# mx-mark/VideoTransformer-pytorch

Hardware: AMD Instinct MI355X
Metric: clips/sec TimeSformer-B divided_space_time 8x3x224x224 fwd+bwd (whole job) (higher is better)
Workload: dtype bf16

## Files before the change

### videotransformer-pytorch_amd/csrc/gemm_nt.hip

```cpp
#include "gemm_common.h"

namespace vtx {

constexpr int BK16 = 64;

__global__ __launch_bounds__(NT_THREADS) void gemm_nt_bf16_kernel(
    int M, int N, int K, const bf16raw* __restrict__ A, long lda, vtx_rowmap amap,
    const bf16raw* __restrict__ B, long ldb, int tiles_n, EpiParams ep) {
  extern __shared__ __attribute__((aligned(16))) char smem[];
  bf16raw* As = reinterpret_cast<bf16raw*>(smem);
  bf16raw* Bs = As + 2 * BM * BK16;
  const int tid = threadIdx.x, lane = tid & 63, wave = tid >> 6;
  const int wm = wave >> 1, wn = wave & 1;
  const int nwg = gridDim.x;
  const int tile = xcd_remap(blockIdx.x, nwg);
  const int tm = tile / tiles_n, tn = tile - tm * tiles_n;
  const int m0 = tm * BM, n0 = tn * BN;

  const int lc = tid & 7, lr = tid >> 3;
  const bf16raw* ap[4];
  const bf16raw* bp[4];
  int lds_off[4];
#pragma unroll
  for (int it = 0; it < 4; ++it) {
// ... 291 lines not shown
constexpr int PP_RING_BYTES = 2 * PP_BUF * 2;
constexpr int PP_STG_LD = 64;
constexpr int PP_LDS_BYTES = PP_RING_BYTES + 8 * 16 * PP_STG_LD * 4;
constexpr int PP_GRID = 256;

__device__ inline void lgkm0() { asm volatile("s_waitcnt lgkmcnt(0)" ::: "memory"); }

enum { PRE_NONE = 0, PRE_RES = 1, PRE_DGELU = 2, PRE_MUL = 3 };
template <bool EPI2, int PRE, bool HAS_SC, bool HAS_ACT, bool CONT, bool ROLL = false>
__global__ __launch_bounds__(PP_THREADS, 2) void gemm_nt_bf16_pp_kernel(
    int M, int N, int K, const bf16raw* __restrict__ A, long lda, vtx_rowmap amap,
    const bf16raw* __restrict__ B, long ldb, int tiles_n, int tiles_total, int CG, int* __restrict__ tile_ctr,
    long long* __restrict__ trace, int dbg, EpiParams ep) {
  extern __shared__ __attribute__((aligned(16))) char smem[];
  bf16raw* lds = reinterpret_cast<bf16raw*>(smem);
  amap.tab = nullptr;
  const int tid = threadIdx.x, lane = tid & 63;
  const int wave = __builtin_amdgcn_readfirstlane(tid >> 6);
  const int wr = wave >> 2, wc = wave & 3;
  float* stg = reinterpret_cast<float*>(smem + PP_RING_BYTES) + wave * 16 * PP_STG_LD;
  const int nk = K / PP_BK;
  int trace_tile = 0;
  auto stamp = [&](int e) {
    if (trace != nullptr && tid == 0 && trace_tile < 8) {
      long long* slot = trace + ((long)blockIdx.x * 8 + trace_tile) * 16;
      slot[e] = (long long)__builtin_amdgcn_s_memrealtime();
      if (e == 1 || e == 2) slot[7 + e] = (long long)__builtin_amdgcn_s_memtime();
    }
  };

// ... 19 lines not shown
  auto publish = [&](int v) -> int {
    if (tid == 0) *bcast = v;
    lgkm0();
    __builtin_amdgcn_s_barrier();
    const int t = *bcast;
    lgkm0();
    __builtin_amdgcn_s_barrier();
    return __builtin_amdgcn_readfirstlane(t);
  };
  auto next_tile = [&]() -> int {
    int v = 0;
    if (tid == 0) v = atomicAdd(my_ctr, 1);
    return publish(v);
  };
  static_assert(!CONT || EPI2, "the continuous flows belong to the read-ahead epilogue");
  constexpr bool CF = CONT && PRE == PRE_NONE;
  constexpr bool PF = CONT && PRE != PRE_NONE;
  const char* abase = nullptr;
  const char* bbase = nullptr;
  unsigned off[4][2];
  int m0 = 0, n0 = 0;
  int m0s = 0, n0s = 0;
  int par = 0;
  auto set_tile = [&](int t, long koff) {
    const int grp_tiles = nrow * CG;
    const int g = t / grp_tiles;
    const int wg = min(CG, tiles_n - g * CG);
    const int r = t - g * grp_tiles;
    const int rr = r / wg, cc = r - rr * wg;
    const int tm = rlo + rr, tn = g * CG + cc;
    m0s = tm * PP_BM; n0s = tn * PP_BN;
    const TileMap am = make_tile_map(amap, m0s);
// ... 98 lines not shown
      PP_READ_A(buf, 3);                                                                               \
      H3_                                                                                              \
      lgkm0();                                                                                         \
      PP_BAR();                                                                                        \
      PP_MMA_H(2, 1, fb1, ISS_(1, kt + 2, e2), M3W_, M3B_);                                            \
      PP_BAR();                                                                                        \
                                 \
      if (W4_) { if (w2) { if (X4_) wait_vmcnt<8 + NST>(); else if (R4_) wait_vmcnt<10>(); else wait_vmcnt<8>(); } else if (w1) wait_vmcnt<4>(); } \
      H4_                                                                                              \
      PP_BAR();                                                                                        \
      PP_MMA_H(2, 0, fb0, ISS_(2, kt + 2, e2), M4W_, M4B_);                                            \
      PP_BAR();                                                                                        \
    }
#define PP_ISS_COND(kind_, ktv_, ex_) if (ex_) issue(kind_, ktv_)
#define PP_ISS_ALWAYS(kind_, ktv_, ex_) issue(kind_, ktv_)
#define PP_ISS_PRE(kind_, ktv_, ex_) if (ex_) issue(kind_, ktv_); else pre_slot(kind_, ktv_)

  typedef __attribute__((address_space(3))) char lds_char;
  const unsigned slot_rd = (unsigned)(unsigned long)(lds_char*)(smem + PP_RING_BYTES);
  const unsigned bias_rd = (unsigned)(unsigned long)(lds_char*)(reinterpret_cast<char*>(stg) + 256 + (lane & 31) * 4);
  constexpr int NST = HAS_ACT ? 32 : 16;
  constexpr int NSR = NST / 4;
  bool relax = false;
  bool prev_rolled = false;
  int t = next_tile();
  const int tend = xcount;
  if (t >= tend) { check_out(); return; }
  int t_next = tend, t_nn = tend;
  if constexpr (CF) t_next = next_tile();
  int pending = 0;
  if (EPI2 && !CF && tid == 0) pending = atomicAdd(my_ctr, 1);
  set_tile(t, 0);
  m0 = m0s; n0 = n0s;
  prologue();
  while (true) {
    f32x16 acc[4][2];
#pragma unroll
    for (int i = 0; i < 4; ++i)
#pragma unroll
      for (int j = 0; j < 2; ++j)
#pragma unroll
        for (int r = 0; r < 16; ++r) acc[i][j][r] = 0.f;
    bf16x8 fa[2][4], fb0[4], fb1[4];
    const bool more_c = CF && t_next < tend;
    const int em0 = m0 + wr * 128, en0 = n0 + wc * 64;
    const int tile_m0 = m0;
    TileMap cm;
    unsigned ldcb = 0, lean_skipb = 0;
    bool lean = false;
    [[maybe_unused]] bool rolled = false;
    int lean_lb = 0;
    const char* lean_cb = nullptr;
    [[maybe_unused]] __amdgpu_buffer_rsrc_t lean_rsrc;
    float bcol[2] = {0.f, 0.f};
    auto epi_head = [&]() {
      cm = make_tile_map(ep.cmap, tile_m0);
      ldcb = (unsigned)ep.ldc * 2u;
      const long skipb64 = (long)cm.skip * (long)ldcb;
      lean = CONT && (dbg == 0 || dbg == 5 || dbg == 6) && em0 + 127 < ep.M && en0 + 63 < ep.N && (ep.split_row <= 0 || em0 + 127 < ep.split_row) &&
// ... 48 lines not shown
      _Pragma("unroll") for (int u = 0; u < 2; ++u) {                                                   \
        const unsigned sel = u ? 0x07060302u : 0x05040100u;                                             \
        u32x4 o;                                                                                        \
        o[0] = __builtin_amdgcn_perm(pl_w0[1], pl_w0[0], sel);                                          \
        o[1] = __builtin_amdgcn_perm(pl_w0[3], pl_w0[2], sel);                                          \
        o[2] = __builtin_amdgcn_perm(pl_w1[1], pl_w1[0], sel);                                          \
        o[3] = __builtin_amdgcn_perm(pl_w1[3], pl_w1[2], sel);                                          \
        const unsigned voff = pl_v0 + (u ? ldcb : 0u) + ((2 * pl_p2 + u >= lean_lb - 16 * (p_)) ? lean_skipb : 0u); \
         \
         \
        if constexpr (ROLL) __builtin_amdgcn_raw_buffer_store_b128(o, lean_rsrc, voff + (unsigned)(16 * (p_)) * ldcb, 0, 2); \
        else st16_nt_b(base, voff, o);                                                                  \
      }                                                                                                 \
    }
    constexpr bool ROLLK = ROLL;
    static_assert(!ROLL || (CF && VTX_PP_BF16_STAGE && PRE == PRE_NONE && !HAS_SC && !HAS_ACT), "rolling: the plain continuous flow only");
    stamp(0);
    if (relax) wait_vmcnt<10 + NST>(); else wait_vmcnt<10>();
    PP_BAR();
    stamp(1);
    if (wr == 1) PP_BAR();
    if constexpr (CF) {
      auto bias_dma = [&]() {
        if (ep.bias) {
          const int c = n0 + wc * 64 + lane;
          __builtin_amdgcn_global_load_lds((const __attribute__((address_space(1))) void*)(ep.bias + (c < ep.N ? c : 0)),
                                           (__attribute__((address_space(3))) void*)(stg + 64), 4, 0, 0);
        }
        if constexpr (HAS_SC) {
#pragma unroll
          for (int h = 0; h < 2; ++h) {
            int ml = m0 + wr * 128 + h * 64 + lane;
            if (ml >= ep.M) ml = ep.M - 1;
            const bool split = ep.split_row > 0 && ml >= ep.split_row;
            const unsigned q1 = fast_div((unsigned)ml, ep.rs_magic1, ep.rs_shift1);
            const unsigned q2 = fast_div((unsigned)ml, ep.rs_magic2, ep.rs_shift2);
            const int idx = split ? (ml - ep.split_row) : (int)q1 * ep.rs_m1 + (ml - (int)q2 * ep.rs_d2) * ep.rs_m2;
// ... 38 lines not shown
                      , PP_PF(0) PP_PW(0, 1) PP_PR();,
                      PP_PWAIT(0);, PP_PF(2) PP_PW(1, 1) PP_PR();)
        } else {
          PP_KTILE_XH(true, true, true, true, true, PP_ISS_ALWAYS, PP_CF_H1, PP_CF_H2;, PP_CF_H3, PP_CF_H4,
                      relax && kt < 2, relax && kt == 0, relax && kt == 0, prev_rolled && kt == 1, false, , , , )
        }
#undef PP_CF_H1
#undef PP_CF_H2
#undef PP_CF_H3
#undef PP_CF_H4
      } else {
        for (; kt < nk; ++kt) {
          PP_KTILE(kt + 1 < nk, kt + 2 < nk, kt + 1 < nk, kt + 2 < nk, true, PP_ISS_COND, if (kt == 0) bias_dma();, , , )
        }
      }
    } else if constexpr (PF) {
      constexpr bool pres = PRE == PRE_RES;
      const int pen = n0 + wc * 64 + (lane & 7) * 8;
      const unsigned penc2 = pen < ep.N ? (unsigned)pen * 2u : 0u;
      const unsigned pld2 = (unsigned)(pres ? ep.ldr : ep.ld_dgelu) * 2u;
      const int lastv = min(ep.M - 1, (pres && ep.split_row > 0) ? ep.split_row - 1 : 0x7fffffff);
      const int m0c = min(m0, lastv);
      const TileMap prm = make_tile_map(ep.rmap, m0c);
      const long pfirst = pres ? tile_map_row_u(prm, ep.rmap, m0c) : (long)m0c;
      const char* pbase = reinterpret_cast<const char*>(pres ? ep.R : ep.dgelu_in) + pfirst * (long)pld2;
      const int pbl = (pres && ep.rmap.grp > 0) ? prm.bound - m0c : 0x7fffffff;
      const int pskip = pres ? prm.skip : 0;
      const int plast = lastv - m0c;
      const int pl0 = (m0 - m0c) + wr * 128 + (lane >> 3);
      auto pre_piece = [&](int j, bf16raw* dst) {
        const int l = min(pl0 + 8 * j, plast);
        const int lr = l + (l >= pbl ? pskip : 0);
        const char* b = pbase;
        asm volatile("" : "+s"(b));
        dma16_nt(reinterpret_cast<const bf16raw*>(b + ((unsigned)lr * pld2 + penc2)), dst);
      };
      auto pre_slot = [&](int kind, int ktv) {
        const int s = (ktv - nk) * 4 + kind;
        bf16raw* dst = lds + ((ktv & 1) ^ par) * PP_BUF + kind * PP_REGION + wave * 1024;
        pre_piece(2 * s, dst);
        pre_piece(2 * s + 1, dst + 512);
        if (s == 6) {
          bf16raw* dst7 = lds + ((ktv & 1) ^ par) * PP_BUF + 3 * PP_REGION + wave * 1024;
          pre_piece(14, dst7);
          pre_piece(15, dst7 + 512);
        }
      };
      for (int kt = 0; kt < nk; ++kt) {
        PP_KTILE(kt + 1 < nk, kt + 2 < nk, true, true, kt + 1 < nk, PP_ISS_PRE, , , , )
      }
    } else {
      for (int kt = 0; kt < nk; ++kt) {
        PP_KTILE(kt + 1 < nk, kt + 2 < nk, kt + 1 < nk, kt + 2 < nk, true, PP_ISS_COND, , , , )
      }
    }
    if (wr == 0) PP_BAR();
    stamp(2);
    if constexpr (!EPI2) {
      t = next_tile();
      const bool more = t < tend;
      if (more) { set_tile(t, 0); m0 = m0s; n0 = n0s; prologue(); }
#define PP_EPI(mi_, half_)                                                                              \
      {                                                                                                 \
        const int col = lane & 31, rhalf = (lane >> 5) * 4;                                             \
        _Pragma("unroll") for (int ni = 0; ni < 2; ++ni) _Pragma("unroll") for (int r = 0; r < 8; ++r)  \
            stg[((r & 3) + 8 * (r >> 2) + rhalf) * PP_STG_LD + ni * 32 + col] = acc[mi_][ni][8 * (half_) + r]; \
        lgkm0();                                                                                        \
        __builtin_amdgcn_wave_barrier();                                                                \
        epilogue<bf16raw, 16, 2, PP_STG_LD>(ep, stg, em0 + (mi_) * 32 + (half_) * 16, en0, lane);       \
        lgkm0();                                                                                        \
        __builtin_amdgcn_wave_barrier();                                                                \
      }
      PP_EPI(0, 0) PP_EPI(0, 1) PP_EPI(1, 0) PP_EPI(1, 1) PP_EPI(2, 0) PP_EPI(2, 1) PP_EPI(3, 0) PP_EPI(3, 1)
#undef PP_EPI
      if (!more) break;
    } else {
      bool more = more_c;
      if constexpr (!CF) {
        t = publish(pending);
        more = t < tend;
      }
      stamp(3);
      int le = lane;
      asm volatile("" : "+v"(le));
      const int en = en0 + (le & 7) * 8;
      const bool col_ok = en < ep.N;
      const int enc = col_ok ? en : 0;
      const int er = em0 + (le >> 3);
      constexpr bool HAS_PRE = PRE != PRE_NONE, pre_res = PRE == PRE_RES;
      bf16raw* const pre_lds = lds + wave * (128 * 64);
      if (!rolled) epi_head();
      if constexpr (HAS_PRE && !PF) {
        const bf16raw* const pre_base = reinterpret_cast<const bf16raw*>(pre_res ? ep.R : ep.dgelu_in);
        const long pre_ld = pre_res ? ep.ldr : ep.ld_dgelu;
        const TileMap rm = make_tile_map(ep.rmap, tile_m0);
        const int row_last = ep.M - 1;
#pragma unroll
        for (int j = 0; j < 16; ++j) {
          int ml = er + 8 * j;
          const bool past = ml > row_last;
          if (past) ml = row_last;
          long rr = ml;
          if (pre_res) {
            const bool split = ep.split_row > 0 && ml >= ep.split_row;
            rr = split ? 0 : (ep.r_period > 0 ? (long)(ml % ep.r_period) : (past ? map_row(ep.rmap, ml) : tile_map_row(rm, ep.rmap, ml)));
          }
          dma16(pre_base + rr * pre_ld + enc, pre_lds + j * 512);
        }
      }
      if (ep.bias && !rolled) {
        if constexpr (CF) {
          asm volatile("ds_read_b32 %0, %2\n\tds_read_b32 %1, %2 offset:128\n\ts_waitcnt lgkmcnt(0)"
                       : "=&v"(bcol[0]), "=&v"(bcol[1]) : "v"(bias_rd) : "memory");
        } else {
#pragma unroll
          for (int ni = 0; ni < 2; ++ni) {
            const int c = en0 + ni * 32 + (le & 31);
            bcol[ni] = ep.bias[c < ep.N ? c : 0];
          }
        }
      }
      float sc[8][2];
      float scl[2] = {0.f, 0.f};
      if constexpr (HAS_SC && CF) {
        if (lean) {
          const unsigned scl_rd = (unsigned)(unsigned long)(lds_char*)(reinterpret_cast<char*>(stg) + 512 + le * 4);
          asm volatile("ds_read_b32 %0, %2\n\tds_read_b32 %1, %2 offset:256\n\ts_waitcnt lgkmcnt(0)"
                       : "=&v"(scl[0]), "=&v"(scl[1]) : "v"(scl_rd) : "memory");
        } else {
        const unsigned sc_rd = (unsigned)(unsigned long)(lds_char*)(reinterpret_cast<char*>(stg) + 512 + (le >> 3) * 4);
        asm volatile("ds_read_b32 %0, %16\n\tds_read_b32 %1, %16 offset:32\n\tds_read_b32 %2, %16 offset:64\n\t"
                     "ds_read_b32 %3, %16 offset:96\n\tds_read_b32 %4, %16 offset:128\n\tds_read_b32 %5, %16 offset:160\n\t"
                     "ds_read_b32 %6, %16 offset:192\n\tds_read_b32 %7, %16 offset:224\n\tds_read_b32 %8, %16 offset:256\n\t"
                     "ds_read_b32 %9, %16 offset:288\n\tds_read_b32 %10, %16 offset:320\n\tds_read_b32 %11, %16 offset:352\n\t"
                     "ds_read_b32 %12, %16 offset:384\n\tds_read_b32 %13, %16 offset:416\n\tds_read_b32 %14, %16 offset:448\n\t"
                     "ds_read_b32 %15, %16 offset:480\n\ts_waitcnt lgkmcnt(0)"
                     : "=&v"(sc[0][0]), "=&v"(sc[0][1]), "=&v"(sc[1][0]), "=&v"(sc[1][1]), "=&v"(sc[2][0]), "=&v"(sc[2][1]),
                       "=&v"(sc[3][0]), "=&v"(sc[3][1]), "=&v"(sc[4][0]), "=&v"(sc[4][1]), "=&v"(sc[5][0]), "=&v"(sc[5][1]),
                       "=&v"(sc[6][0]), "=&v"(sc[6][1]), "=&v"(sc[7][0]), "=&v"(sc[7][1])
                     : "v"(sc_rd) : "memory");
        }
      }
      if constexpr (HAS_SC && !CF) {
        auto scale_of = [&](int ml) -> float {
          if (ml >= ep.M) ml = ep.M - 1;
          const bool split = ep.split_row > 0 && ml >= ep.split_row;
          const unsigned q1 = fast_div((unsigned)ml, ep.rs_magic1, ep.rs_shift1);
          const unsigned q2 = fast_div((unsigned)ml, ep.rs_magic2, ep.rs_shift2);
          return ep.row_scale[split ? (ml - ep.split_row) : (int)q1 * ep.rs_m1 + (ml - (int)q2 * ep.rs_d2) * ep.rs_m2];
        };
        if (lean) {
          scl[0] = scale_of(em0 + le);
          scl[1] = scale_of(em0 + 64 + le);
        } else {
#pragma unroll
          for (int p = 0; p < 8; ++p)
#pragma unroll
            for (int u = 0; u < 2; ++u) sc[p][u] = scale_of(er + 16 * p + 8 * u);
        }
      }
      if constexpr (!CF) {
        if (more && tid == 0) pending = atomicAdd(my_ctr, 1);
        asm volatile("s_waitcnt vmcnt(0)" ::: "memory");
        stamp(4);
        asm volatile("" : "+v"(bcol[0]));
        asm volatile("" : "+v"(bcol[1]));
        if constexpr (HAS_SC) {
#pragma unroll
          for (int p = 0; p < 8; ++p) { asm volatile("" : "+v"(sc[p][0])); asm volatile("" : "+v"(sc[p][1])); }
          asm volatile("" : "+v"(scl[0])); asm volatile("" : "+v"(scl[1]));
        }
        if constexpr (!HAS_PRE) {
          if (more) { set_tile(t, 0); m0 = m0s; n0 = n0s; prologue(); }
        }
        if constexpr (PF) {
          if (more) set_tile(t, (long)nk * (PP_BK * 2));
        }
      }
      stamp(5);
      const unsigned stg_rd = (unsigned)(unsigned long)(lds_char*)(reinterpret_cast<char*>(stg) +
                                                                    ((le >> 3) * PP_STG_LD + (le & 7) * 8) * 4);
      const unsigned pre_rd = (unsigned)(unsigned long)(lds_char*)(reinterpret_cast<char*>(pre_lds) + le * 16);
      const unsigned pf_rd = (unsigned)(unsigned long)(lds_char*)(reinterpret_cast<char*>(lds + wave * 1024) + le * 16);
      const int pa = (nk & 1) ^ par;
#define PP_EPI2(p_, mi_, half_)                                                                         \
      {                                                                                                 \
        const int col = le & 31, rhalf = (le >> 5) * 4;                                             \
        if (dbg != 3) {                                                                                 \
        _Pragma("unroll") for (int ni = 0; ni < 2; ++ni) _Pragma("unroll") for (int r = 0; r < 8; ++r)  \
            stg[((r & 3) + 8 * (r >> 2) + rhalf) * PP_STG_LD + ni * 32 + col] = acc[mi_][ni][8 * (half_) + r] + bcol[ni]; \
        } else { stg[le] = acc[mi_][0][8 * (half_)] + acc[mi_][1][8 * (half_) + 7]; }                 \
        lgkm0();                                                                                        \
        __builtin_amdgcn_wave_barrier();                                                                \
        f32x4 s00, s01, s10, s11;                                                                       \
        u32x4 pre[2];                                                                                   \
        if constexpr (HAS_PRE) {                                                                        \
          const unsigned prd__ = PF ? pf_rd + (unsigned)((((p_) < 4 ? pa : pa ^ 1) * PP_BUF + ((p_) & 3) * PP_REGION) * 2) \
                                    : pre_rd + 2 * (p_) * 1024;                                         \
          asm volatile("ds_read_b128 %0, %6\n\tds_read_b128 %1, %6 offset:16\n\t"                       \
                       "ds_read_b128 %2, %6 offset:2048\n\tds_read_b128 %3, %6 offset:2064\n\t"         \
                       "ds_read_b128 %4, %7\n\tds_read_b128 %5, %7 offset:1024\n\t"                     \
                       "s_waitcnt lgkmcnt(0)"                                                           \
                       : "=&v"(s00), "=&v"(s01), "=&v"(s10), "=&v"(s11), "=&v"(pre[0]), "=&v"(pre[1])   \
                       : "v"(stg_rd), "v"(prd__) : "memory");                                           \
        } else                                                                                            \
          asm volatile("ds_read_b128 %0, %4\n\tds_read_b128 %1, %4 offset:16\n\t"                       \
                       "ds_read_b128 %2, %4 offset:2048\n\tds_read_b128 %3, %4 offset:2064\n\t"         \
                       "s_waitcnt lgkmcnt(0)"                                                           \
                       : "=&v"(s00), "=&v"(s01), "=&v"(s10), "=&v"(s11) : "v"(stg_rd) : "memory");      \
        __builtin_amdgcn_sched_barrier(0);                                                              \
        float v[2][8];                                                                                  \
        _Pragma("unroll") for (int j = 0; j < 4; ++j) {                                                 \
          v[0][j] = s00[j]; v[0][4 + j] = s01[j]; v[1][j] = s10[j]; v[1][4 + j] = s11[j];               \
        }                                                                                               \
        _Pragma("unroll") for (int u = 0; u < 2; ++u) {                                                 \
          const int m = er + 16 * (p_) + 8 * u;                                                         \
          const bool ok = col_ok && m < ep.M && dbg != 2;                                               \
          const bool split = ep.split_row > 0 && m >= ep.split_row;                                     \
          if constexpr (HAS_ACT) {                                                                      \
            if (ep.act == 2) {                               \
              float gp[8];                                                                              \
              _Pragma("unroll") for (int j = 0; j < 8; ++j) gelu_erf_both(v[u][j], v[u][j], gp[j]);     \
              if (ok) PP_ST8(reinterpret_cast<bf16raw*>(ep.C2) + (long)m * ep.ldc2 + en, gp);        \
            } else {                                                                                    \
              if (ep.C2 && ok) store8(reinterpret_cast<bf16raw*>(ep.C2) + (long)m * ep.ldc2 + en, v[u]); \
              _Pragma("unroll") for (int j = 0; j < 8; ++j) v[u][j] = gelu_erf(v[u][j]);                \
            }                                                                                           \
          }                                                                                             \
          if constexpr (PRE == PRE_MUL) {                          \
            const uint32_t w[4] = {pre[u][0], pre[u][1], pre[u][2], pre[u][3]};                         \
            _Pragma("unroll") for (int j = 0; j < 4; ++j) {                                             \
              v[u][2 * j] *= __uint_as_float(w[j] << 16);                                               \
              v[u][2 * j + 1] *= __uint_as_float(w[j] & 0xffff0000u);                                   \
            }                                                                                           \
          }                                                                                             \
          if constexpr (PRE == PRE_DGELU) {                                                             \
            const uint32_t w[4] = {pre[u][0], pre[u][1], pre[u][2], pre[u][3]};                         \
            _Pragma("unroll") for (int j = 0; j < 4; ++j) {                                             \
              v[u][2 * j] *= gelu_erf_grad(__uint_as_float(w[j] << 16));                                \
              v[u][2 * j + 1] *= gelu_erf_grad(__uint_as_float(w[j] & 0xffff0000u));                    \
            }                                                                                           \
          }                                                                                             \
          if constexpr (HAS_SC) { _Pragma("unroll") for (int j = 0; j < 8; ++j) v[u][j] *= sc[p_][u]; } \
          if (pre_res && !split) {                                                                      \
            const uint32_t w[4] = {pre[u][0], pre[u][1], pre[u][2], pre[u][3]};                         \
            _Pragma("unroll") for (int j = 0; j < 4; ++j) {                                             \
              v[u][2 * j] += __uint_as_float(w[j] << 16);                                               \
              v[u][2 * j + 1] += __uint_as_float(w[j] & 0xffff0000u);                                   \
            }                                                                                           \
          }                                                                                             \
          if (ok) {                                                                                     \
            if (split) store8(reinterpret_cast<bf16raw*>(ep.Csplit) + (long)(m - ep.split_row) * ep.ldsplit + en, v[u]); \
            else PP_ST8(reinterpret_cast<bf16raw*>(ep.C) + tile_map_row(cm, ep.cmap, m) * ep.ldc + en, v[u]); \
          }                                                                                             \
        }                                                                                               \
        if constexpr (PF) {                         \
          if ((p_) < 7 && more) issue((p_) & 3, nk + ((p_) >> 2));                                      \
        }                                                                                               \
      }
      constexpr bool PAIRS = VTX_PP_BF16_STAGE && PRE == PRE_NONE && !HAS_SC && !HAS_ACT;
      const unsigned stg_wr0 = (unsigned)(unsigned long)(lds_char*)(reinterpret_cast<char*>(stg)) ;
      if (lean) {
        int ln = le;
        asm volatile("" : "+v"(ln));
        if constexpr (PAIRS) {
          if (rolled) {
            PP_PWAIT(0); PP_PF(3)
          } else {
            pl_setup();
            PP_PW(0, 0) PP_PR();
            PP_PW(0, 1) PP_PWAIT(4); PP_PF(0) PP_PR();
            PP_PW(1, 0) PP_PWAIT(4); PP_PF(1) PP_PR();
// ... 3 lines not shown
          PP_PW(2, 0) PP_PR();
          PP_PW(2, 1) PP_PWAIT(4); PP_PF(4) PP_PR();
          PP_PW(3, 0) PP_PWAIT(4); PP_PF(5) PP_PR();
          PP_PW(3, 1) PP_PWAIT(4); PP_PF(6) PP_PR();
          PP_PWAIT(0); PP_PF(7)
        } else {
          const unsigned wa0 = stg_wr0 + (unsigned)(((ln >> 5) * 256 + (ln & 31)) * 4), wa1 = wa0 + 512 * 4;
          const unsigned vf0 = (unsigned)(ln >> 3) * ldcb + (unsigned)(ln & 7) * 16u;
          const unsigned ldc2b = (unsigned)ep.ldc2 * 2u;
          const unsigned vg0 = (unsigned)(ln >> 3) * ldc2b + (unsigned)(ln & 7) * 16u;
          const char* const lean_c2b = reinterpret_cast<const char*>(ep.C2) + ((long)em0 * ep.ldc2 + en0) * 2;
          f32x4 s00, s01, s10, s11;
          u32x4 pre[2];
          float scu[2] = {1.f, 1.f};
          const unsigned bp_addr = (unsigned)(ln >> 3) * 4u;
#define PP_LW(mi_, half_) if (ep.bias) { PP_LW_(mi_, half_, true) } else { PP_LW_(mi_, half_, false) }
#define PP_LW_(mi_, half_, B_)                                                                          \
          {                                                                                             \
            _Pragma("unroll") for (int kk = 0; kk < 2; ++kk) _Pragma("unroll") for (int ni = 0; ni < 2; ++ni) \
            _Pragma("unroll") for (int r2 = 0; r2 < 2; ++r2) {                                          \
              f32x2 xy = mk2(acc[mi_][ni][8 * (half_) + 4 * kk + 2 * r2], acc[mi_][ni][8 * (half_) + 4 * kk + 2 * r2 + 1]); \
              if (B_) { const f32x2 b2 = mk2(bcol[ni], bcol[ni]); xy = xy + b2; }                       \
              const float x = xy[0];                                                                    \
              const float y = xy[1];                                                                    \
              const unsigned wa = kk ? wa1 : wa0;                                                       \
              if (ni == 0 && r2 == 0) asm volatile("ds_write2_b32 %0, %1, %2 offset1:64" :: "v"(wa), "v"(x), "v"(y) : "memory"); \
              if (ni == 0 && r2 == 1) asm volatile("ds_write2_b32 %0, %1, %2 offset0:128 offset1:192" :: "v"(wa), "v"(x), "v"(y) : "memory"); \
              if (ni == 1 && r2 == 0) asm volatile("ds_write2_b32 %0, %1, %2 offset0:32 offset1:96" :: "v"(wa), "v"(x), "v"(y) : "memory"); \
              if (ni == 1 && r2 == 1) asm volatile("ds_write2_b32 %0, %1, %2 offset0:160 offset1:224" :: "v"(wa), "v"(x), "v"(y) : "memory"); \
            }                                                                                           \
          }
#define PP_LR(p_)                                                                                       \
          if constexpr (HAS_PRE) {                                                                      \
            const unsigned prd__ = PF ? pf_rd + (unsigned)((((p_) < 4 ? pa : pa ^ 1) * PP_BUF + ((p_) & 3) * PP_REGION) * 2) \
                                      : pre_rd + 2 * (p_) * 1024;                                       \
            asm volatile("ds_read_b128 %0, %6\n\tds_read_b128 %1, %6 offset:16\n\t"                     \
                         "ds_read_b128 %2, %6 offset:2048\n\tds_read_b128 %3, %6 offset:2064\n\t"       \
                         "ds_read_b128 %4, %7\n\tds_read_b128 %5, %7 offset:1024"                       \
                         : "=&v"(s00), "=&v"(s01), "=&v"(s10), "=&v"(s11), "=&v"(pre[0]), "=&v"(pre[1]) \
                         : "v"(stg_rd), "v"(prd__) : "memory");                                         \
          } else                                                                                        \
            asm volatile("ds_read_b128 %0, %4\n\tds_read_b128 %1, %4 offset:16\n\t"                     \
                         "ds_read_b128 %2, %4 offset:2048\n\tds_read_b128 %3, %4 offset:2064"           \
                         : "=&v"(s00), "=&v"(s01), "=&v"(s10), "=&v"(s11) : "v"(stg_rd) : "memory");      \
          if constexpr (HAS_SC)                         \
            asm volatile("ds_bpermute_b32 %0, %2, %3 offset:%4\n\tds_bpermute_b32 %1, %2, %3 offset:%5"   \
                         : "=&v"(scu[0]), "=&v"(scu[1]) : "v"(bp_addr), "v"((p_) < 4 ? scl[0] : scl[1]),   \
                           "n"(((16 * (p_)) & 63) * 4), "n"(((16 * (p_) + 8) & 63) * 4) : "memory")
#define PP_LWAITF(n_)                                                                                   \
          if constexpr (HAS_PRE) { PP_LWAIT(n_, "+v"(s00), "+v"(s01), "+v"(s10), "+v"(s11), "+v"(pre[0]), "+v"(pre[1]), "+v"(scu[0]), "+v"(scu[1])); } \
          else { PP_LWAIT(n_, "+v"(s00), "+v"(s01), "+v"(s10), "+v"(s11), "+v"(scu[0]), "+v"(scu[1])); }
#define PP_LF(p_)                                                                                       \
          {                                                                                             \
            _Pragma("clang fp contract(off)")         \
            float v[2][8];                                                                              \
            _Pragma("unroll") for (int j = 0; j < 4; ++j) {                                             \
              v[0][j] = s00[j]; v[0][4 + j] = s01[j]; v[1][j] = s10[j]; v[1][4 + j] = s11[j];           \
            }                                                                                           \
            const char* const base = lean_cb + (long)(16 * (p_)) * ldcb;                                \
            _Pragma("unroll") for (int u = 0; u < 2; ++u) {                                             \
              if constexpr (HAS_ACT) {                       \
                float gp[8];                                                                            \
                _Pragma("unroll") for (int j = 0; j < 8; ++j) gelu_erf_both(v[u][j], v[u][j], gp[j]);   \
                st16_nt_s(lean_c2b + (long)(16 * (p_)) * ldc2b, vg0 + (u ? 8u * ldc2b : 0u), pack8(gp)); \
              }                                                                                         \
              if constexpr (PRE == PRE_MUL) {                      \
                const uint32_t w[4] = {pre[u][0], pre[u][1], pre[u][2], pre[u][3]};                     \
                _Pragma("unroll") for (int j = 0; j < 4; ++j) {                                         \
                  v[u][2 * j] *= __uint_as_float(w[j] << 16);                                           \
                  v[u][2 * j + 1] *= __uint_as_float(w[j] & 0xffff0000u);                               \
                }                                                                                       \
              }                                                                                         \
              if constexpr (HAS_SC) { _Pragma("unroll") for (int j = 0; j < 8; ++j) v[u][j] *= scu[u]; } \
              if constexpr (pre_res) {                               \
                const uint32_t w[4] = {pre[u][0], pre[u][1], pre[u][2], pre[u][3]};                     \
                _Pragma("unroll") for (int j = 0; j < 4; ++j) {                                         \
                  v[u][2 * j] += __uint_as_float(w[j] << 16);                                           \
                  v[u][2 * j + 1] += __uint_as_float(w[j] & 0xffff0000u);                               \
                }                                                                                       \
              }                                                                                         \
              const unsigned voff = vf0 + (u ? 8u * ldcb : 0u) +                                        \
                                    (((ln >> 3) + 8 * u >= lean_lb - 16 * (p_)) ? lean_skipb : 0u);   \
              st16_nt_s(base, voff, pack8(v[u]));                                                       \
            }                                                                                           \
            if constexpr (PF) {                       \
              if ((p_) < 7 && more) issue((p_) & 3, nk + ((p_) >> 2));                                  \
            }                                                                                           \
          }
          PP_LW(0, 0) PP_LR(0);
          PP_LW(0, 1) PP_LWAITF(8) PP_LF(0) PP_LR(1);
          PP_LW(1, 0) PP_LWAITF(8) PP_LF(1) PP_LR(2);
          PP_LW(1, 1) PP_LWAITF(8) PP_LF(2) PP_LR(3);
          PP_LW(2, 0) PP_LWAITF(8) PP_LF(3) PP_LR(4);
          PP_LW(2, 1) PP_LWAITF(8) PP_LF(4) PP_LR(5);
          PP_LW(3, 0) PP_LWAITF(8) PP_LF(5) PP_LR(6);
          PP_LW(3, 1) PP_LWAITF(8) PP_LF(6) PP_LR(7);
          PP_LWAITF(0) PP_LF(7)
#undef PP_LW
#undef PP_LW_
#undef PP_LR
#undef PP_LWAITF
// ... 31 lines not shown
            o[3] = __builtin_amdgcn_perm(w1[3], w1[2], sel);                                            \
            const int m = em0 + 16 * (p_) + 2 * p2 + u;                                                 \
            const bool ok = col_ok && m < ep.M && dbg != 2;                                             \
            const bool split = ep.split_row > 0 && m >= ep.split_row;                                   \
            if (ok) {                                                                                   \
              if (split) *reinterpret_cast<u32x4*>(reinterpret_cast<bf16raw*>(ep.Csplit) + (long)(m - ep.split_row) * ep.ldsplit + en) = o; \
              else __builtin_nontemporal_store(o, reinterpret_cast<u32x4*>(reinterpret_cast<bf16raw*>(ep.C) + tile_map_row(cm, ep.cmap, m) * ep.ldc + en)); \
            }                                                                                           \
          }                                                                                             \
          __builtin_amdgcn_wave_barrier();                                                              \
        }
        PP_EPI2B(0, 0, 0) PP_EPI2B(1, 0, 1) PP_EPI2B(2, 1, 0) PP_EPI2B(3, 1, 1)
        PP_EPI2B(4, 2, 0) PP_EPI2B(5, 2, 1) PP_EPI2B(6, 3, 0) PP_EPI2B(7, 3, 1)
#undef PP_EPI2B
      } else {
        PP_EPI2(0, 0, 0) PP_EPI2(1, 0, 1) PP_EPI2(2, 1, 0) PP_EPI2(3, 1, 1)
        PP_EPI2(4, 2, 0) PP_EPI2(5, 2, 1) PP_EPI2(6, 3, 0) PP_EPI2(7, 3, 1)
      }
#undef PP_EPI2
      stamp(6);
      if constexpr (HAS_PRE && !PF) {
        __builtin_amdgcn_s_barrier();
        if (more) { set_tile(t, 0); m0 = m0s; n0 = n0s; prologue(); }
      }
      stamp(7);
      ++trace_tile;
      if (!more) break;
      if constexpr (CONT) {
        abase += (long)nk * (PP_BK * 2); bbase += (long)nk * (PP_BK * 2);
        if constexpr (CF) {
          const bool second = !HAS_ACT || ep.act == 2 || ep.C2 != nullptr;
          relax = em0 + 120 < ep.M && en0 < ep.N && second && trace == nullptr && (dbg == 0 || dbg == 4 || dbg == 5 || dbg == 6) && nk >= 3;
          prev_rolled = rolled;
        }
        m0 = m0s; n0 = n0s;
        par ^= nk & 1;
        if constexpr (CF) { t = t_next; t_next = t_nn; }
      }
    }
  }
  check_out();
#undef PP_KTILE
#undef PP_LWAIT
#undef PP_PWAIT
#undef PP_PW
#undef PP_PW_
#undef PP_PR
#undef PP_PF
#undef PP_ISS_COND
#undef PP_ISS_ALWAYS
#undef PP_ISS_PRE
#undef PP_READ_A
#undef PP_READ_B
#undef PP_MMA
#undef PP_BAR
}

template <bool EPI2, int PRE, bool HAS_SC, bool HAS_ACT, bool CONT, bool ROLL = false>
static int launch_pp_t(const vtx_gemm_desc* d, const EpiParams& ep, hipStream_t st, const Options& cfg) {
  allow_lds<gemm_nt_bf16_pp_kernel<EPI2, PRE, HAS_SC, HAS_ACT, CONT, ROLL>>(PP_LDS_BYTES, PP_LDS_BYTES);
  const int tiles_m = cdiv(d->M, PP_BM), tiles_n = cdiv(d->N, PP_BN);
  int cg = cfg.pp_cg ? cfg.pp_cg : (int)(6291456L / (512L * d->K));
  if (!cfg.pp_cg && cg < 3) cg = 3;
  if (!cfg.pp_cg && cg > 6) cg = 6;
  if (cg < 1) cg = 1;
  hipLaunchKernelGGL((gemm_nt_bf16_pp_kernel<EPI2, PRE, HAS_SC, HAS_ACT, CONT, ROLL>), dim3(cfg.pp_grid), dim3(PP_THREADS), PP_LDS_BYTES, st, d->M, d->N, d->K,
// ... 5 lines not shown
static int launch_pp(const vtx_gemm_desc* d, const EpiParams& ep, hipStream_t st) {
  const Options& cfg = options();
  if (cfg.pp_epi == 1) return launch_pp_t<false, PRE_NONE, false, false, false>(d, ep, st, cfg);
  const bool sc = d->row_scale != nullptr;
  const bool cont = cfg.pp_cont != 0 && (d->amap.grp <= 0 || d->amap.grp >= 256) && d->K / PP_BK >= 3;
  if (d->act) return cont ? launch_pp_t<true, PRE_NONE, false, true, true>(d, ep, st, cfg) : launch_pp_t<true, PRE_NONE, false, true, false>(d, ep, st, cfg);
  if (d->dgelu_in) {
    if (d->dgelu_kind == 1)
      return cont && 256L * d->ld_dgelu * 2 < (1L << 31) ? launch_pp_t<true, PRE_MUL, false, false, true>(d, ep, st, cfg) : launch_pp_t<true, PRE_MUL, false, false, false>(d, ep, st, cfg);
    return launch_pp_t<true, PRE_DGELU, false, false, false>(d, ep, st, cfg);
  }
  if (d->R) {
    const bool pf = cont && d->r_period <= 0 && (d->rmap.grp <= 0 || d->rmap.grp >= 256) && d->rmap.skip >= 0 &&
                    (256L + (d->rmap.skip > 0 ? d->rmap.skip : 0)) * d->ldr * 2 < (1L << 31);
    if (!pf) return sc ? launch_pp_t<true, PRE_RES, true, false, false>(d, ep, st, cfg) : launch_pp_t<true, PRE_RES, false, false, false>(d, ep, st, cfg);
    if (sc) return cont ? launch_pp_t<true, PRE_RES, true, false, true>(d, ep, st, cfg) : launch_pp_t<true, PRE_RES, true, false, false>(d, ep, st, cfg);
    return cont ? launch_pp_t<true, PRE_RES, false, false, true>(d, ep, st, cfg) : launch_pp_t<true, PRE_RES, false, false, false>(d, ep, st, cfg);
  }
  if (sc) return cont ? launch_pp_t<true, PRE_NONE, true, false, true>(d, ep, st, cfg) : launch_pp_t<true, PRE_NONE, true, false, false>(d, ep, st, cfg);
  const bool roll = cont && cfg.pp_epi == 6 && d->K / PP_BK >= 4 && d->N % 64 == 0 && d->split_row <= 0 && closed_form(d->cmap) &&
                    (d->cmap.grp <= 0 || d->cmap.grp >= 256) && d->cmap.skip >= 0 && d->ldc < (1L << 22) &&
                    (long)(d->cmap.grp > 0 ? d->cmap.skip : 0) * d->ldc * 2 < (1L << 30);
  if (roll) return launch_pp_t<true, PRE_NONE, false, false, true, true>(d, ep, st, cfg);
  return cont ? launch_pp_t<true, PRE_NONE, false, false, true>(d, ep, st, cfg) : launch_pp_t<true, PRE_NONE, false, false, false>(d, ep, st, cfg);
}

constexpr int BK32 = 16;
constexpr int LD32 = BK32 + 1;

__global__ __launch_bounds__(NT_THREADS) void gemm_nt_f32_kernel(
    int M, int N, int K, const float* __restrict__ A, long lda, vtx_rowmap amap,
    const float* __restrict__ B, long ldb, int tiles_n, EpiParams ep) {
// ... 174 lines not shown
```

Before: 749.8.

## Load epilogue pre-operands into registers in continuous persistent GEMM

```diff
diff --git a/videotransformer-pytorch_amd/csrc/gemm_nt.hip b/videotransformer-pytorch_amd/csrc/gemm_nt.hip
--- a/videotransformer-pytorch_amd/csrc/gemm_nt.hip
+++ b/videotransformer-pytorch_amd/csrc/gemm_nt.hip
@@ -329,6 +329,8 @@
     long long* __restrict__ trace, int dbg, EpiParams ep) {
   extern __shared__ __attribute__((aligned(16))) char smem[];
   bf16raw* lds = reinterpret_cast<bf16raw*>(smem);
+  constexpr bool PREG = CONT && PRE != PRE_NONE;
+  static_assert(!CONT || PRE != PRE_DGELU, "the GELU' input kernel is never continuous");
   amap.tab = nullptr;
   const int tid = threadIdx.x, lane = tid & 63;
   const int wave = __builtin_amdgcn_readfirstlane(tid >> 6);
@@ -378,8 +380,6 @@
     return publish(v);
   };
   static_assert(!CONT || EPI2, "the continuous flows belong to the read-ahead epilogue");
-  constexpr bool CF = CONT && PRE == PRE_NONE;
-  constexpr bool PF = CONT && PRE != PRE_NONE;
   const char* abase = nullptr;
   const char* bbase = nullptr;
   unsigned off[4][2];
@@ -508,7 +508,6 @@
     }
 #define PP_ISS_COND(kind_, ktv_, ex_) if (ex_) issue(kind_, ktv_)
 #define PP_ISS_ALWAYS(kind_, ktv_, ex_) issue(kind_, ktv_)
-#define PP_ISS_PRE(kind_, ktv_, ex_) if (ex_) issue(kind_, ktv_); else pre_slot(kind_, ktv_)
 
   typedef __attribute__((address_space(3))) char lds_char;
   const unsigned slot_rd = (unsigned)(unsigned long)(lds_char*)(smem + PP_RING_BYTES);
@@ -521,9 +520,9 @@
   const int tend = xcount;
   if (t >= tend) { check_out(); return; }
   int t_next = tend, t_nn = tend;
-  if constexpr (CF) t_next = next_tile();
+  if constexpr (CONT) t_next = next_tile();
   int pending = 0;
-  if (EPI2 && !CF && tid == 0) pending = atomicAdd(my_ctr, 1);
+  if (EPI2 && !CONT && tid == 0) pending = atomicAdd(my_ctr, 1);
   set_tile(t, 0);
   m0 = m0s; n0 = n0s;
   prologue();
@@ -536,7 +535,13 @@
 #pragma unroll
         for (int r = 0; r < 16; ++r) acc[i][j][r] = 0.f;
     bf16x8 fa[2][4], fb0[4], fb1[4];
-    const bool more_c = CF && t_next < tend;
+    if constexpr (PREG) {
+      int lf = lane;
+      asm volatile("" : "+v"(lf));
+#pragma unroll
+      for (int ks = 0; ks < 4; ++ks) fr[ks] = (lf & 31) * PP_BK + (((2 * ks + (lf >> 5)) ^ (((lf & 31) >> 1) & 7)) << 3);
+    }
+    const bool more_c = CONT && t_next < tend;
     const int em0 = m0 + wr * 128, en0 = n0 + wc * 64;
     const int tile_m0 = m0;
     TileMap cm;
@@ -615,13 +620,13 @@
       }                                                                                                 \
     }
     constexpr bool ROLLK = ROLL;
-    static_assert(!ROLL || (CF && VTX_PP_BF16_STAGE && PRE == PRE_NONE && !HAS_SC && !HAS_ACT), "rolling: the plain continuous flow only");
+    static_assert(!ROLL || (CONT && VTX_PP_BF16_STAGE && PRE == PRE_NONE && !HAS_SC && !HAS_ACT), "rolling: the plain continuous flow only");
     stamp(0);
     if (relax) wait_vmcnt<10 + NST>(); else wait_vmcnt<10>();
     PP_BAR();
     stamp(1);
     if (wr == 1) PP_BAR();
-    if constexpr (CF) {
+    if constexpr (CONT) {
       auto bias_dma = [&]() {
         if (ep.bias) {
           const int c = n0 + wc * 64 + lane;
@@ -690,41 +695,6 @@
           PP_KTILE(kt + 1 < nk, kt + 2 < nk, kt + 1 < nk, kt + 2 < nk, true, PP_ISS_COND, if (kt == 0) bias_dma();, , , )
         }
       }
-    } else if constexpr (PF) {
-      constexpr bool pres = PRE == PRE_RES;
-      const int pen = n0 + wc * 64 + (lane & 7) * 8;
-      const unsigned penc2 = pen < ep.N ? (unsigned)pen * 2u : 0u;
-      const unsigned pld2 = (unsigned)(pres ? ep.ldr : ep.ld_dgelu) * 2u;
-      const int lastv = min(ep.M - 1, (pres && ep.split_row > 0) ? ep.split_row - 1 : 0x7fffffff);
-      const int m0c = min(m0, lastv);
-      const TileMap prm = make_tile_map(ep.rmap, m0c);
-      const long pfirst = pres ? tile_map_row_u(prm, ep.rmap, m0c) : (long)m0c;
-      const char* pbase = reinterpret_cast<const char*>(pres ? ep.R : ep.dgelu_in) + pfirst * (long)pld2;
-      const int pbl = (pres && ep.rmap.grp > 0) ? prm.bound - m0c : 0x7fffffff;
-      const int pskip = pres ? prm.skip : 0;
-      const int plast = lastv - m0c;
-      const int pl0 = (m0 - m0c) + wr * 128 + (lane >> 3);
-      auto pre_piece = [&](int j, bf16raw* dst) {
-        const int l = min(pl0 + 8 * j, plast);
-        const int lr = l + (l >= pbl ? pskip : 0);
-        const char* b = pbase;
-        asm volatile("" : "+s"(b));
-        dma16_nt(reinterpret_cast<const bf16raw*>(b + ((unsigned)lr * pld2 + penc2)), dst);
-      };
-      auto pre_slot = [&](int kind, int ktv) {
-        const int s = (ktv - nk) * 4 + kind;
-        bf16raw* dst = lds + ((ktv & 1) ^ par) * PP_BUF + kind * PP_REGION + wave * 1024;
-        pre_piece(2 * s, dst);
-        pre_piece(2 * s + 1, dst + 512);
-        if (s == 6) {
-          bf16raw* dst7 = lds + ((ktv & 1) ^ par) * PP_BUF + 3 * PP_REGION + wave * 1024;
-          pre_piece(14, dst7);
-          pre_piece(15, dst7 + 512);
-        }
-      };
-      for (int kt = 0; kt < nk; ++kt) {
-        PP_KTILE(kt + 1 < nk, kt + 2 < nk, true, true, kt + 1 < nk, PP_ISS_PRE, , , , )
-      }
     } else {
       for (int kt = 0; kt < nk; ++kt) {
         PP_KTILE(kt + 1 < nk, kt + 2 < nk, kt + 1 < nk, kt + 2 < nk, true, PP_ISS_COND, , , , )
@@ -752,7 +722,7 @@
       if (!more) break;
     } else {
       bool more = more_c;
-      if constexpr (!CF) {
+      if constexpr (!CONT) {
         t = publish(pending);
         more = t < tend;
       }
@@ -766,7 +736,32 @@
       constexpr bool HAS_PRE = PRE != PRE_NONE, pre_res = PRE == PRE_RES;
       bf16raw* const pre_lds = lds + wave * (128 * 64);
       if (!rolled) epi_head();
-      if constexpr (HAS_PRE && !PF) {
+      [[maybe_unused]] u32x4 blk[16];
+      auto blk_load = [&]() {
+        const unsigned penc2 = col_ok ? (unsigned)en * 2u : 0u;
+        const unsigned pld2 = (unsigned)(pre_res ? ep.ldr : ep.ld_dgelu) * 2u;
+        const int lastv = min(ep.M - 1, (pre_res && ep.split_row > 0) ? ep.split_row - 1 : 0x7fffffff);
+        const int m0c = min(tile_m0, lastv);
+        const TileMap prm = make_tile_map(ep.rmap, m0c);
+        const long pfirst = pre_res ? tile_map_row_u(prm, ep.rmap, m0c) : (long)m0c;
+        const char* pbase = reinterpret_cast<const char*>(pre_res ? ep.R : ep.dgelu_in) + pfirst * (long)pld2;
+        asm volatile("" : "+s"(pbase));
+        const int pbl = (pre_res && ep.rmap.grp > 0) ? prm.bound - m0c : 0x7fffffff;
+        const int pskip = pre_res ? prm.skip : 0;
+        const int plast = lastv - m0c;
+        const int pl0 = (tile_m0 - m0c) + wr * 128 + (le >> 3);
+#pragma unroll
+        for (int j = 0; j < 16; ++j) {
+          const int l = min(pl0 + 8 * j, plast);
+          const int lr = l + (l >= pbl ? pskip : 0);
+          const unsigned vo = (unsigned)lr * pld2 + penc2;
+          asm volatile("global_load_dwordx4 %0, %1, %2 nt" : "=v"(blk[j]) : "v"(vo), "s"(pbase) : "memory");
+        }
+      };
+#define PP_BLOAD() if constexpr (PREG) blk_load()
+#define PP_BLK(p_, u_) (PREG ? blk[2 * (p_) + (u_)] : pre[u_])
+#define PP_BWAIT(p_) if constexpr (PREG) { asm volatile("s_waitcnt vmcnt(%2)" : "+v"(blk[2 * (p_)]), "+v"(blk[2 * (p_) + 1]) : "n"(14 - 2 * (p_)) : "memory"); }
+      if constexpr (HAS_PRE && !CONT) {
         const bf16raw* const pre_base = reinterpret_cast<const bf16raw*>(pre_res ? ep.R : ep.dgelu_in);
         const long pre_ld = pre_res ? ep.ldr : ep.ld_dgelu;
         const TileMap rm = make_tile_map(ep.rmap, tile_m0);
@@ -785,7 +780,7 @@
         }
       }
       if (ep.bias && !rolled) {
-        if constexpr (CF) {
+        if constexpr (CONT) {
           asm volatile("ds_read_b32 %0, %2\n\tds_read_b32 %1, %2 offset:128\n\ts_waitcnt lgkmcnt(0)"
                        : "=&v"(bcol[0]), "=&v"(bcol[1]) : "v"(bias_rd) : "memory");
         } else {
@@ -798,8 +793,8 @@
       }
       float sc[8][2];
       float scl[2] = {0.f, 0.f};
-      if constexpr (HAS_SC && CF) {
-        if (lean) {
+      if constexpr (HAS_SC && CONT) {
+        if (lean || PREG) {
           const unsigned scl_rd = (unsigned)(unsigned long)(lds_char*)(reinterpret_cast<char*>(stg) + 512 + le * 4);
           asm volatile("ds_read_b32 %0, %2\n\tds_read_b32 %1, %2 offset:256\n\ts_waitcnt lgkmcnt(0)"
                        : "=&v"(scl[0]), "=&v"(scl[1]) : "v"(scl_rd) : "memory");
@@ -817,7 +812,7 @@
                      : "v"(sc_rd) : "memory");
         }
       }
-      if constexpr (HAS_SC && !CF) {
+      if constexpr (HAS_SC && !CONT) {
         auto scale_of = [&](int ml) -> float {
           if (ml >= ep.M) ml = ep.M - 1;
           const bool split = ep.split_row > 0 && ml >= ep.split_row;
@@ -835,7 +830,7 @@
             for (int u = 0; u < 2; ++u) sc[p][u] = scale_of(er + 16 * p + 8 * u);
         }
       }
-      if constexpr (!CF) {
+      if constexpr (!CONT) {
         if (more && tid == 0) pending = atomicAdd(my_ctr, 1);
         asm volatile("s_waitcnt vmcnt(0)" ::: "memory");
         stamp(4);
@@ -849,30 +844,37 @@
         if constexpr (!HAS_PRE) {
           if (more) { set_tile(t, 0); m0 = m0s; n0 = n0s; prologue(); }
         }
-        if constexpr (PF) {
-          if (more) set_tile(t, (long)nk * (PP_BK * 2));
-        }
       }
       stamp(5);
       const unsigned stg_rd = (unsigned)(unsigned long)(lds_char*)(reinterpret_cast<char*>(stg) +
                                                                     ((le >> 3) * PP_STG_LD + (le & 7) * 8) * 4);
       const unsigned pre_rd = (unsigned)(unsigned long)(lds_char*)(reinterpret_cast<char*>(pre_lds) + le * 16);
-      const unsigned pf_rd = (unsigned)(unsigned long)(lds_char*)(reinterpret_cast<char*>(lds + wave * 1024) + le * 16);
-      const int pa = (nk & 1) ^ par;
+      const int kpar = nk & 1;
 #define PP_EPI2(p_, mi_, half_)                                                                         \
       {                                                                                                 \
-        const int col = le & 31, rhalf = (le >> 5) * 4;                                             \
+         \
+         \
+        int lp = le;                                                                                    \
+        if constexpr (PREG) asm volatile("" : "+v"(lp));                                                \
+        const int enp = PREG ? en0 + (lp & 7) * 8 : en, erp = PREG ? em0 + (lp >> 3) : er;              \
+        const bool cokp = PREG ? enp < ep.N : col_ok;                                                   \
+        const int col = lp & 31, rhalf = (lp >> 5) * 4;                                                 \
         if (dbg != 3) {                                                                                 \
         _Pragma("unroll") for (int ni = 0; ni < 2; ++ni) _Pragma("unroll") for (int r = 0; r < 8; ++r)  \
             stg[((r & 3) + 8 * (r >> 2) + rhalf) * PP_STG_LD + ni * 32 + col] = acc[mi_][ni][8 * (half_) + r] + bcol[ni]; \
-        } else { stg[le] = acc[mi_][0][8 * (half_)] + acc[mi_][1][8 * (half_) + 7]; }                 \
+        } else { stg[lp] = acc[mi_][0][8 * (half_)] + acc[mi_][1][8 * (half_) + 7]; }                 \
         lgkm0();                                                                                        \
         __builtin_amdgcn_wave_barrier();                                                                \
         f32x4 s00, s01, s10, s11;                                                                       \
         u32x4 pre[2];                                                                                   \
-        if constexpr (HAS_PRE) {                                                                        \
-          const unsigned prd__ = PF ? pf_rd + (unsigned)((((p_) < 4 ? pa : pa ^ 1) * PP_BUF + ((p_) & 3) * PP_REGION) * 2) \
-                                    : pre_rd + 2 * (p_) * 1024;                                         \
+        PP_BWAIT(p_)                                                                                    \
+        [[maybe_unused]] float scp[2];                \
+        if constexpr (HAS_SC && PREG)                                                                   \
+          asm volatile("ds_bpermute_b32 %0, %2, %3 offset:%4\n\tds_bpermute_b32 %1, %2, %3 offset:%5\n\ts_waitcnt lgkmcnt(0)" \
+                       : "=&v"(scp[0]), "=&v"(scp[1]) : "v"((unsigned)(lp >> 3) * 4u), "v"((p_) < 4 ? scl[0] : scl[1]), \
+                         "n"(((16 * (p_)) & 63) * 4), "n"(((16 * (p_) + 8) & 63) * 4) : "memory");     \
+        if constexpr (HAS_PRE && !PREG) {                                                               \
+          const unsigned prd__ = pre_rd + 2 * (p_) * 1024;                                              \
           asm volatile("ds_read_b128 %0, %6\n\tds_read_b128 %1, %6 offset:16\n\t"                       \
                        "ds_read_b128 %2, %6 offset:2048\n\tds_read_b128 %3, %6 offset:2064\n\t"         \
                        "ds_read_b128 %4, %7\n\tds_read_b128 %5, %7 offset:1024\n\t"                     \
@@ -890,48 +892,46 @@
           v[0][j] = s00[j]; v[0][4 + j] = s01[j]; v[1][j] = s10[j]; v[1][4 + j] = s11[j];               \
         }                                                                                               \
         _Pragma("unroll") for (int u = 0; u < 2; ++u) {                                                 \
-          const int m = er + 16 * (p_) + 8 * u;                                                         \
-          const bool ok = col_ok && m < ep.M && dbg != 2;                                               \
+          const int m = erp + 16 * (p_) + 8 * u;                                                        \
+          const bool ok = cokp && m < ep.M && dbg != 2;                                                 \
           const bool split = ep.split_row > 0 && m >= ep.split_row;                                     \
           if constexpr (HAS_ACT) {                                                                      \
             if (ep.act == 2) {                               \
               float gp[8];                                                                              \
               _Pragma("unroll") for (int j = 0; j < 8; ++j) gelu_erf_both(v[u][j], v[u][j], gp[j]);     \
-              if (ok) PP_ST8(reinterpret_cast<bf16raw*>(ep.C2) + (long)m * ep.ldc2 + en, gp);        \
+              if (ok) PP_ST8(reinterpret_cast<bf16raw*>(ep.C2) + (long)m * ep.ldc2 + enp, gp);          \
             } else {                                                                                    \
-              if (ep.C2 && ok) store8(reinterpret_cast<bf16raw*>(ep.C2) + (long)m * ep.ldc2 + en, v[u]); \
+              if (ep.C2 && ok) store8(reinterpret_cast<bf16raw*>(ep.C2) + (long)m * ep.ldc2 + enp, v[u]); \
               _Pragma("unroll") for (int j = 0; j < 8; ++j) v[u][j] = gelu_erf(v[u][j]);                \
             }                                                                                           \
           }                                                                                             \
           if constexpr (PRE == PRE_MUL) {                          \
-            const uint32_t w[4] = {pre[u][0], pre[u][1], pre[u][2], pre[u][3]};                         \
+            const u32x4 w = PP_BLK(p_, u);                                                              \
             _Pragma("unroll") for (int j = 0; j < 4; ++j) {                                             \
               v[u][2 * j] *= __uint_as_float(w[j] << 16);                                               \
               v[u][2 * j + 1] *= __uint_as_float(w[j] & 0xffff0000u);                                   \
             }                                                                                           \
           }                                                                                             \
           if constexpr (PRE == PRE_DGELU) {                                                             \
-            const uint32_t w[4] = {pre[u][0], pre[u][1], pre[u][2], pre[u][3]};                         \
+            const u32x4 w = PP_BLK(p_, u);                                                              \
             _Pragma("unroll") for (int j = 0; j < 4; ++j) {                                             \
               v[u][2 * j] *= gelu_erf_grad(__uint_as_float(w[j] << 16));                                \
               v[u][2 * j + 1] *= gelu_erf_grad(__uint_as_float(w[j] & 0xffff0000u));                    \
             }                                                                                           \
           }                                                                                             \
-          if constexpr (HAS_SC) { _Pragma("unroll") for (int j = 0; j < 8; ++j) v[u][j] *= sc[p_][u]; } \
+          if constexpr (HAS_SC && !PREG) { _Pragma("unroll") for (int j = 0; j < 8; ++j) v[u][j] *= sc[p_][u]; } \
+          if constexpr (HAS_SC && PREG) { _Pragma("unroll") for (int j = 0; j < 8; ++j) v[u][j] *= scp[u]; } \
           if (pre_res && !split) {                                                                      \
-            const uint32_t w[4] = {pre[u][0], pre[u][1], pre[u][2], pre[u][3]};                         \
+            const u32x4 w = PP_BLK(p_, u);                                                              \
             _Pragma("unroll") for (int j = 0; j < 4; ++j) {                                             \
               v[u][2 * j] += __uint_as_float(w[j] << 16);                                               \
               v[u][2 * j + 1] += __uint_as_float(w[j] & 0xffff0000u);                                   \
             }                                                                                           \
           }                                                                                             \
           if (ok) {                                                                                     \
-            if (split) store8(reinterpret_cast<bf16raw*>(ep.Csplit) + (long)(m - ep.split_row) * ep.ldsplit + en, v[u]); \
-            else PP_ST8(reinterpret_cast<bf16raw*>(ep.C) + tile_map_row(cm, ep.cmap, m) * ep.ldc + en, v[u]); \
+            if (split) store8(reinterpret_cast<bf16raw*>(ep.Csplit) + (long)(m - ep.split_row) * ep.ldsplit + enp, v[u]); \
+            else PP_ST8(reinterpret_cast<bf16raw*>(ep.C) + tile_map_row(cm, ep.cmap, m) * ep.ldc + enp, v[u]); \
           }                                                                                             \
-        }                                                                                               \
-        if constexpr (PF) {                         \
-          if ((p_) < 7 && more) issue((p_) & 3, nk + ((p_) >> 2));                                      \
         }                                                                                               \
       }
       constexpr bool PAIRS = VTX_PP_BF16_STAGE && PRE == PRE_NONE && !HAS_SC && !HAS_ACT;
@@ -965,6 +965,7 @@
           u32x4 pre[2];
           float scu[2] = {1.f, 1.f};
           const unsigned bp_addr = (unsigned)(ln >> 3) * 4u;
+          PP_BLOAD();
 #define PP_LW(mi_, half_) if (ep.bias) { PP_LW_(mi_, half_, true) } else { PP_LW_(mi_, half_, false) }
 #define PP_LW_(mi_, half_, B_)                                                                          \
           {                                                                                             \
@@ -982,9 +983,8 @@
             }                                                                                           \
           }
 #define PP_LR(p_)                                                                                       \
-          if constexpr (HAS_PRE) {                                                                      \
-            const unsigned prd__ = PF ? pf_rd + (unsigned)((((p_) < 4 ? pa : pa ^ 1) * PP_BUF + ((p_) & 3) * PP_REGION) * 2) \
-                                      : pre_rd + 2 * (p_) * 1024;                                       \
+          if constexpr (HAS_PRE && !PREG) {                                                             \
+            const unsigned prd__ = pre_rd + 2 * (p_) * 1024;                                            \
             asm volatile("ds_read_b128 %0, %6\n\tds_read_b128 %1, %6 offset:16\n\t"                     \
                          "ds_read_b128 %2, %6 offset:2048\n\tds_read_b128 %3, %6 offset:2064\n\t"       \
                          "ds_read_b128 %4, %7\n\tds_read_b128 %5, %7 offset:1024"                       \
@@ -999,11 +999,12 @@
                          : "=&v"(scu[0]), "=&v"(scu[1]) : "v"(bp_addr), "v"((p_) < 4 ? scl[0] : scl[1]),   \
                            "n"(((16 * (p_)) & 63) * 4), "n"(((16 * (p_) + 8) & 63) * 4) : "memory")
 #define PP_LWAITF(n_)                                                                                   \
-          if constexpr (HAS_PRE) { PP_LWAIT(n_, "+v"(s00), "+v"(s01), "+v"(s10), "+v"(s11), "+v"(pre[0]), "+v"(pre[1]), "+v"(scu[0]), "+v"(scu[1])); } \
+          if constexpr (HAS_PRE && !PREG) { PP_LWAIT(n_, "+v"(s00), "+v"(s01), "+v"(s10), "+v"(s11), "+v"(pre[0]), "+v"(pre[1]), "+v"(scu[0]), "+v"(scu[1])); } \
           else { PP_LWAIT(n_, "+v"(s00), "+v"(s01), "+v"(s10), "+v"(s11), "+v"(scu[0]), "+v"(scu[1])); }
 #define PP_LF(p_)                                                                                       \
           {                                                                                             \
             _Pragma("clang fp contract(off)")         \
+            PP_BWAIT(p_)                              \
             float v[2][8];                                                                              \
             _Pragma("unroll") for (int j = 0; j < 4; ++j) {                                             \
               v[0][j] = s00[j]; v[0][4 + j] = s01[j]; v[1][j] = s10[j]; v[1][4 + j] = s11[j];           \
@@ -1016,7 +1017,7 @@
                 st16_nt_s(lean_c2b + (long)(16 * (p_)) * ldc2b, vg0 + (u ? 8u * ldc2b : 0u), pack8(gp)); \
               }                                                                                         \
               if constexpr (PRE == PRE_MUL) {                      \
-                const uint32_t w[4] = {pre[u][0], pre[u][1], pre[u][2], pre[u][3]};                     \
+                const u32x4 w = PP_BLK(p_, u);                                                          \
                 _Pragma("unroll") for (int j = 0; j < 4; ++j) {                                         \
                   v[u][2 * j] *= __uint_as_float(w[j] << 16);                                           \
                   v[u][2 * j + 1] *= __uint_as_float(w[j] & 0xffff0000u);                               \
@@ -1024,7 +1025,7 @@
               }                                                                                         \
               if constexpr (HAS_SC) { _Pragma("unroll") for (int j = 0; j < 8; ++j) v[u][j] *= scu[u]; } \
               if constexpr (pre_res) {                               \
-                const uint32_t w[4] = {pre[u][0], pre[u][1], pre[u][2], pre[u][3]};                     \
+                const u32x4 w = PP_BLK(p_, u);                                                          \
                 _Pragma("unroll") for (int j = 0; j < 4; ++j) {                                         \
                   v[u][2 * j] += __uint_as_float(w[j] << 16);                                           \
                   v[u][2 * j + 1] += __uint_as_float(w[j] & 0xffff0000u);                               \
@@ -1033,9 +1034,6 @@
               const unsigned voff = vf0 + (u ? 8u * ldcb : 0u) +                                        \
                                     (((ln >> 3) + 8 * u >= lean_lb - 16 * (p_)) ? lean_skipb : 0u);   \
               st16_nt_s(base, voff, pack8(v[u]));                                                       \
-            }                                                                                           \
-            if constexpr (PF) {                       \
-              if ((p_) < 7 && more) issue((p_) & 3, nk + ((p_) >> 2));                                  \
             }                                                                                           \
           }
           PP_LW(0, 0) PP_LR(0);
@@ -1097,12 +1095,16 @@
         PP_EPI2B(4, 2, 0) PP_EPI2B(5, 2, 1) PP_EPI2B(6, 3, 0) PP_EPI2B(7, 3, 1)
 #undef PP_EPI2B
       } else {
+        PP_BLOAD();
         PP_EPI2(0, 0, 0) PP_EPI2(1, 0, 1) PP_EPI2(2, 1, 0) PP_EPI2(3, 1, 1)
         PP_EPI2(4, 2, 0) PP_EPI2(5, 2, 1) PP_EPI2(6, 3, 0) PP_EPI2(7, 3, 1)
       }
 #undef PP_EPI2
+#undef PP_BWAIT
+#undef PP_BLOAD
+#undef PP_BLK
       stamp(6);
-      if constexpr (HAS_PRE && !PF) {
+      if constexpr (HAS_PRE && !CONT) {
         __builtin_amdgcn_s_barrier();
         if (more) { set_tile(t, 0); m0 = m0s; n0 = n0s; prologue(); }
       }
@@ -1111,14 +1113,12 @@
       if (!more) break;
       if constexpr (CONT) {
         abase += (long)nk * (PP_BK * 2); bbase += (long)nk * (PP_BK * 2);
-        if constexpr (CF) {
-          const bool second = !HAS_ACT || ep.act == 2 || ep.C2 != nullptr;
-          relax = em0 + 120 < ep.M && en0 < ep.N && second && trace == nullptr && (dbg == 0 || dbg == 4 || dbg == 5 || dbg == 6) && nk >= 3;
-          prev_rolled = rolled;
-        }
+        const bool second = !HAS_ACT || ep.act == 2 || ep.C2 != nullptr;
+        relax = em0 + 120 < ep.M && en0 < ep.N && second && trace == nullptr && (dbg == 0 || dbg == 4 || dbg == 5 || dbg == 6) && nk >= 3;
+        prev_rolled = rolled;
         m0 = m0s; n0 = n0s;
-        par ^= nk & 1;
-        if constexpr (CF) { t = t_next; t_next = t_nn; }
+        par ^= kpar;
+        t = t_next; t_next = t_nn;
       }
     }
   }
@@ -1132,7 +1132,6 @@
 #undef PP_PF
 #undef PP_ISS_COND
 #undef PP_ISS_ALWAYS
-#undef PP_ISS_PRE
 #undef PP_READ_A
 #undef PP_READ_B
 #undef PP_MMA
@@ -1168,8 +1167,7 @@
     const bool pf = cont && d->r_period <= 0 && (d->rmap.grp <= 0 || d->rmap.grp >= 256) && d->rmap.skip >= 0 &&
                     (256L + (d->rmap.skip > 0 ? d->rmap.skip : 0)) * d->ldr * 2 < (1L << 31);
     if (!pf) return sc ? launch_pp_t<true, PRE_RES, true, false, false>(d, ep, st, cfg) : launch_pp_t<true, PRE_RES, false, false, false>(d, ep, st, cfg);
-    if (sc) return cont ? launch_pp_t<true, PRE_RES, true, false, true>(d, ep, st, cfg) : launch_pp_t<true, PRE_RES, true, false, false>(d, ep, st, cfg);
-    return cont ? launch_pp_t<true, PRE_RES, false, false, true>(d, ep, st, cfg) : launch_pp_t<true, PRE_RES, false, false, false>(d, ep, st, cfg);
+    return sc ? launch_pp_t<true, PRE_RES, true, false, true>(d, ep, st, cfg) : launch_pp_t<true, PRE_RES, false, false, true>(d, ep, st, cfg);
   }
   if (sc) return cont ? launch_pp_t<true, PRE_NONE, true, false, true>(d, ep, st, cfg) : launch_pp_t<true, PRE_NONE, true, false, false>(d, ep, st, cfg);
   const bool roll = cont && cfg.pp_epi == 6 && d->K / PP_BK >= 4 && d->N % 64 == 0 && d->split_row <= 0 && closed_form(d->cmap) &&
```

New measurement: 757.3 (median of 6 runs). 1.01x the previous value.
